# mrluin/TextualDegRemoval

Measured on AMD Instinct MI355X. Metric: train images/sec (512x512, bs=4/GPU), higher is better.
Workload: dtype f32 (3xbf16-split MFMA: 24-bit operand significands on the full fp32 exponent range, fp32 accumulate; unscaled gradients, no loss scale, no step-skip guard; tensors fp32 -- the MASA-encoder ResidualBlock activations / gradients as three bf16 planes whose sum IS the fp32 value, bit for bit)

## Files before the change

include/tdr.h:

```cpp
#ifndef TDR_H
#define TDR_H
#include <stdint.h>
#ifdef __cplusplus
extern "C" {
#endif

#define TDR_ABI_VERSION 112
int tdr_version(void);
const char* tdr_last_error(void);

typedef struct TdrStepGuard {
    float scale, inv_scale, max_scale;
    int good, growth_interval;
    int step, skipped, finite;
    float bc1, bc2_sqrt;
} TdrStepGuard;

typedef struct TdrConvDesc {
    int N, Cin, H, W;
    int Cout, OH, OW;
    int KH, stride, dil, pad;
    const float* in;  int64_t in_ns;
    int gate;
    const float* kscale; int64_t kscale_ns;
// ... 31 lines not shown
    int64_t total;
    int64_t first_block;
} TdrPackJob;
int tdr_pack_job_init(TdrPackJob* job, const float* w, int Cout, int Cin, int KH, int mode, int fmt, void* wp);
int tdr_pack_weights_multi(const TdrPackJob* jobs_dev, int n_jobs, int64_t total_blocks, void* stream);
int tdr_pack_patches(const float* blk, int B, int G, int C, int BH, int BW, int PH, int PW, int pstep, int dil,
                     int off, float* wp, void* stream);

typedef struct TdrConvP16Desc {
    int N, Cin, H, W, Cout;
    const void* in;
    const void* wp; int Mpad; int wp_fmt;
    const float* bias;
    const float* res32;  int64_t res32_ns;
    const void*  res16;
    const float* mask32; int64_t mask32_ns;
    const void*  mask16;
    int relu;
    float* out32; int64_t out32_ns;
    void*  out16;
} TdrConvP16Desc;
int64_t tdr_p16_bytes(int N, int C, int H, int W);
int tdr_p16_from_f32(const float* src, int64_t src_ns, int N, int C, int H, int W, void* dst, void* stream);
int tdr_p16_to_f32(const void* src, int N, int C, int H, int W, float* dst, int64_t dst_ns, void* stream);
int64_t tdr_p16_bytes_fmt(int N, int C, int H, int W, int fmt);
int tdr_p16_from_f32_fmt(const float* src, int64_t src_ns, int N, int C, int H, int W, void* dst, int fmt, void* stream);
int tdr_p16_to_f32_fmt(const void* src, int N, int C, int H, int W, float* dst, int64_t dst_ns, int fmt, void* stream);
int tdr_conv3x3_p16(const TdrConvP16Desc* d, void* stream);
int tdr_conv3x3_p16_force_cfg(int cfg);
typedef struct TdrWgradP16Desc {
    int N, Cin, H, W, Cout;
    const void* in16;
    const void* dout16;
    float* g;
    float* db;
    float* ws; int64_t ws_floats;
    int fmt;
} TdrWgradP16Desc;
int64_t tdr_wgrad3x3_p16_ws_floats(const TdrWgradP16Desc* d);
int tdr_wgrad3x3_p16(const TdrWgradP16Desc* d, void* stream);

typedef struct TdrWgradDesc {
    int N, Cin, H, W, Cout, OH, OW, KH, stride, pad;
    const float* in;   int64_t in_ns;  int gate;
    const float* dout; int64_t dout_ns;
    float* g;
    float* db;
    int per_image;
    float* ws; int64_t ws_floats;
    int math;
} TdrWgradDesc;
int64_t tdr_wgrad_ws_floats(const TdrWgradDesc* d);
int tdr_conv_wgrad(const TdrWgradDesc* d, void* stream);

typedef struct TdrWg1GroupEntry {
    const float* in; const float* dout; float* part; float* dbpart; float* g; float* db;
} TdrWg1GroupEntry;
int tdr_wgrad1x1_group_supported(const TdrWgradDesc* d);
int64_t tdr_wgrad1x1_group_ws_floats(const TdrWgradDesc* d, int nprob);
int tdr_wgrad1x1_group(const TdrWgradDesc* d, int nprob, const void* table, void* stream);

int64_t tdr_wgrad3x3_p16_group_ws_floats(const TdrWgradP16Desc* d, int nprob);
int tdr_wgrad3x3_p16_group_plan(const TdrWgradP16Desc* d, int nprob, int* nsplit, int* units, int* units_per_wg);
int tdr_wgrad3x3_p16_group(const TdrWgradP16Desc* d, int nprob, const void* table, void* stream);

int tdr_layernorm2d_fwd(const float* x, int64_t x_ns, const float* w, const float* b, float eps, int center,
                        int N, int C, int HW, float* y, float* mu, float* rstd, void* stream);
int64_t tdr_ln_ws_floats(int N, int C, int HW);
int tdr_layernorm2d_bwd(const float* go, const float* x, int64_t x_ns, const float* mu, const float* rstd,
                        const float* w, const float* add, int64_t add_ns, int add_C, int center,
                        int N, int C, int HW, float* gx, float* gw, float* gb, float* ws, void* stream);

int64_t tdr_dwsg_ws_floats(int N, int C, int H, int W);
int tdr_dwsg_fwd(const float* t, const float* w, const float* b, int N, int C, int H, int W,
                 float* g, float* pooled, float* ws, void* stream);
int tdr_dwsg_bwd(const float* dg, const float* t, const float* w, const float* b, int N, int C, int H, int W,
                 float* dt, float* dw, float* db, float* ws, void* stream);
int tdr_dwsg_bwd_biased(const float* dg, const float* dg_bias, float dg_bias_mul, const float* t, const float* w, const float* b,
                        int N, int C, int H, int W, float* dt, float* dw, float* db, float* ws, void* stream);
int tdr_dwsg_bwd_parts_supported(int W);
int tdr_dw_param_finish(const float* ws, int N, int C, int H, int W, float* dw , float* db , void* stream);

int tdr_dwgelu_fwd(const float* t, const float* w, const float* b, int N, int C, int H, int W, float* g, void* stream);
int tdr_dwgelu_bwd(const float* dg, const float* t, const float* w, const float* b, int N, int C, int H, int W,
                   float* dt, float* dw, float* db, float* ws, void* stream);
int tdr_dwconv_fwd(const float* t, const float* w, const float* b, int N, int planes, int H, int W, float* out,
                   void* stream);
int tdr_dwconv_bwd(const float* dout, const float* t, const float* w, int N, int planes, int H, int W, float* dt,
                   float* dw, float* db, float* ws, void* stream);
int tdr_dwconv_act_fwd(const float* t, const float* w, const float* b, int N, int planes, int H, int W, int relu, float* out,
                       void* stream);
int tdr_dwconv_act_bwd(const float* dout, const float* act, const float* t, const float* w, int N, int planes, int H, int W,
                       float* dt, float* dw, float* db, float* ws, void* stream);
int tdr_dwpair_fwd(const float* t, const float* w, const float* b, int N, int C, int H, int W, int relu, float* out,
                   int64_t out_ns, void* stream);
int tdr_dwpair_bwd(const float* dout, int64_t dout_ns, const float* act, int64_t act_ns, const float* t, const float* w, int N,
                   int C, int H, int W, float* dt, float* dw, float* db, float* ws, void* stream);
int tdr_dwconv_halves_fwd(const float* t, const float* w, const float* b, int N, int planes, int H, int W, int relu, float* outA,
                          float* outB, int64_t out_ns, void* stream);
int tdr_dwconv_halves_bwd(const float* doutA, const float* doutB, int64_t dout_ns, const float* actA, const float* actB,
                          int64_t act_ns, const float* t, const float* w, int N, int planes, int H, int W, float* dt, float* dw,
                          float* db, float* ws, void* stream);

int tdr_row_sumsq(const float* x, int64_t x_ns, int N, int rows, int HW, float* out, void* stream);
int tdr_mdta_pad(int C);
int tdr_mdta_softmax(const float* G, const float* ss, const float* temp, int N, int C, int heads, float* A, float* AT,
// ... 399 lines not shown
```

textualdegremoval_amd/csrc/tdr_wgrad_1x1.hip:

```cpp
#include "tdr_common.h"
#include "tdr_wgrad_common.h"
#include "../../include/tdr.h"
#include <stdlib.h>

typedef __bf16 g1bf16x8 __attribute__((ext_vector_type(8)));
typedef _Float16 g1f16x8 __attribute__((ext_vector_type(8)));
typedef unsigned g1u32x4 __attribute__((ext_vector_type(4)));

namespace {

enum { G1_BX3 = 0, G1_HX2 = 1 };

constexpr int G1_PX = 32;

template <int SCH>
__device__ __forceinline__ void g1_split8(const f32x4& a, const f32x4& b, g1u32x4 (&p)[SCH == G1_BX3 ? 3 : 2]) {
    if constexpr (SCH == G1_BX3) {
        unsigned h[4], m[4], l[4];
        tdr_split3_bf16<false>(a[0], a[1], h[0], m[0], l[0]);
        tdr_split3_bf16<false>(a[2], a[3], h[1], m[1], l[1]);
        tdr_split3_bf16<false>(b[0], b[1], h[2], m[2], l[2]);
        tdr_split3_bf16<false>(b[2], b[3], h[3], m[3], l[3]);
        p[0] = (g1u32x4){h[0], h[1], h[2], h[3]};
        p[1] = (g1u32x4){m[0], m[1], m[2], m[3]};
// ... 508 lines not shown
    const G1GroupPlan p = g1_group_plan(d, nprob);
    WgArgs a;
    a.in = nullptr; a.in_ns = d->in_ns; a.Cin = d->Cin; a.H = d->H; a.W = d->W;
    a.gate_off = (long)d->Cin * d->H * d->W;
    a.dout = nullptr; a.dout_ns = d->dout_ns; a.Cout = d->Cout; a.OH = d->OH; a.OW = d->OW;
    const G1Tile tl = g1_group_tile(d);
    a.pad = 0; a.tw_log2 = 5; a.tiles_x = tdr_cdiv(d->Cout, 64 * tl.tmw); a.tiles_y = tdr_cdiv(d->Cin, 64 * tl.tnw);
    a.tpi = p.tpi; a.tps = p.tps; a.spi = p.spi;
    a.part = nullptr; a.dbpart = nullptr;
    a.scheme = d->math == 2 ? 1 : 0;
    a.grp_tab = table; a.grp_bpp = p.bpp; a.grp_pairs = nprob * p.bpp;
    hipStream_t st = (hipStream_t)stream;
    const bool g = d->gate != 0;
    int rc;
#define G1_GRP(GATE_, SCH_)                                                                                                       \
    (tl.tmw == 4 ? (tl.tnw == 4 ? launch_grp<GATE_, SCH_, 4, 4>(a, nprob, st) : launch_grp<GATE_, SCH_, 2, 4>(a, nprob, st))      \
                 : (tl.tnw == 2 ? launch_grp<GATE_, SCH_, 2, 2>(a, nprob, st) : launch_grp<GATE_, SCH_, 1, 2>(a, nprob, st)))
    if (a.scheme == 1) rc = g ? G1_GRP(true, G1_HX2) : G1_GRP(false, G1_HX2);
    else rc = g ? G1_GRP(true, G1_BX3) : G1_GRP(false, G1_BX3);
#undef G1_GRP
    if (rc != TDR_OK) return rc;
    const long elems = (long)d->Cout * d->Cin;
    const int nb_main = tdr_cdiv(elems, 256), nb2 = tdr_cdiv(d->Cout, 256);
    hipLaunchKernelGGL(wgrad1x1_grp_reduce_kernel<1>, dim3(nb_main + nb2, nprob), dim3(256), 0, st, static_cast<const TdrWg1GroupEntry*>(table), elems,
                       p.bpp, d->Cout, nb_main);
    TDR_LAUNCH_CHECK("wgrad1x1_grp_reduce_kernel");
    return TDR_OK;
}

namespace {
}

bool tdr_wgrad_1x1_supported(const TdrWgradDesc* d) {
    static const bool off = tdr_tune_env("TDR_WG1") && atoi(tdr_tune_env("TDR_WG1")) == 0;
    if (off || (d->math != 1 && d->math != 2)) return false;
    if (d->KH != 1 || d->stride != 1 || d->pad != 0 || d->H != d->OH || d->W != d->OW) return false;
    const long HW = (long)d->OH * d->OW;
    if (HW % G1_PX != 0 || d->in_ns % 4 != 0 || d->dout_ns % 4 != 0) return false;
    if ((reinterpret_cast<uintptr_t>(d->in) & 15) || (reinterpret_cast<uintptr_t>(d->dout) & 15)) return false;
    return d->Cin >= 64 && d->Cout >= 64;
}

WgPlan tdr_wgrad_1x1_plan(const TdrWgradDesc* d) {
    WgPlan p;
    p.tw_log2 = 5;
    p.cfg = (d->Cout > 64 && d->Cin > 64) ? 0 : 1;
    p.BMc = p.cfg == 0 ? 128 : 64; p.BNc = p.BMc;
    p.WKw = 1;
    const long HW = (long)d->OH * d->OW;
    p.tiles_x = (int)(HW / G1_PX); p.tiles_y = 1;
    p.tpi = p.tiles_x;
    const long out_tiles = (long)tdr_cdiv(d->Cout, p.BMc) * tdr_cdiv(d->Cin, p.BNc);
    static const long want_env = tdr_tune_env("TDR_WG1_WANT") ? atol(tdr_tune_env("TDR_WG1_WANT")) : 0;
    const long want_total = want_env > 0 ? want_env : (d->math == 1 ? 256 : 512);
    long want = want_total / out_tiles;
    if (want < 1) want = 1;
    long spi = (want + d->N - 1) / d->N;
    if (spi > p.tpi / 4) spi = p.tpi / 4;
    if (spi < 1) spi = 1;
    p.tps = tdr_cdiv(p.tpi, spi);
    p.spi = tdr_cdiv(p.tpi, p.tps);
    return p;
}

int tdr_wgrad_1x1_launch(const WgArgs& a, const WgPlan& p, const TdrWgradDesc* d, hipStream_t st) {
    if (p.cfg == 0 && g1_sp() == 1) {
        const bool g = d->gate != 0;
        if (a.scheme == 1) return g ? launch_sp<true, G1_HX2, 2>(a, d->N, st) : launch_sp<false, G1_HX2, 2>(a, d->N, st);
        return g ? launch_sp<true, G1_BX3, 2>(a, d->N, st) : launch_sp<false, G1_BX3, 2>(a, d->N, st);
    }
    if (p.cfg == 0 && g1_sp() == 2) {
        const bool g = d->gate != 0;
        if (a.scheme == 1) return g ? launch_sp<true, G1_HX2, 1>(a, d->N, st) : launch_sp<false, G1_HX2, 1>(a, d->N, st);
        return g ? launch_sp<true, G1_BX3, 1>(a, d->N, st) : launch_sp<false, G1_BX3, 1>(a, d->N, st);
    }
    if (a.scheme == 1) return p.cfg == 0 ? launch_g1_gr<2, 2, G1_HX2>(a, d, st) : launch_g1_gr<1, 1, G1_HX2>(a, d, st);
    return p.cfg == 0 ? launch_g1_gr<2, 2, G1_BX3>(a, d, st) : launch_g1_gr<1, 1, G1_BX3>(a, d, st);
}
```

textualdegremoval_amd/csrc/tdr_wgrad_bx3.hip:

```cpp
#include "tdr_common.h"
#include "tdr_wgrad_common.h"
#include "../../include/tdr.h"

typedef __bf16 bf16x8 __attribute__((ext_vector_type(8)));
typedef _Float16 wf16x8 __attribute__((ext_vector_type(8)));

namespace {

enum { WSCH_BX3 = 0, WSCH_HX2 = 1, WSCH_H1 = 2 };

typedef unsigned u32x4 __attribute__((ext_vector_type(4)));

__device__ __forceinline__ void wsplit3(float x, __bf16& h, __bf16& m, __bf16& l) {
    h = (__bf16)x;
    const float r = x - (float)h;
    m = (__bf16)r;
    l = (__bf16)(r - (float)m);
}

#define WSPLIT_ONE(x, i)                      \
    {                                         \
        __bf16 a0, a1, a2;                    \
        float xp__ = (x);                     \
        asm volatile("" : "+v"(xp__));        \
        wsplit3(xp__, a0, a1, a2);            \
        hv[i] = a0; mv[i] = a1; lv[i] = a2;   \
    }

constexpr int wb_max_nch(int KH, int P) {
    return KH == 3 ? ((P / 32 + 2) * 5 > (P / 8 + 2) * 2 ? ((P / 32 + 2) * 5 > (P / 16 + 2) * 3 ? (P / 32 + 2) * 5 : (P / 16 + 2) * 3)
                                                         : ((P / 8 + 2) * 2 > (P / 16 + 2) * 3 ? (P / 8 + 2) * 2 : (P / 16 + 2) * 3))
                   : P / 8;
}

template <int SCH, bool PIN = true>
__device__ __forceinline__ void split8v(const f32x4& a, const f32x4& b, u32x4& h, u32x4& m, u32x4& l) {
    if constexpr (SCH == WSCH_H1) {
        wf16x8 hv;
#pragma unroll
        for (int i = 0; i < 8; ++i) hv[i] = (_Float16)(i < 4 ? a[i & 3] : b[i & 3]);
        h = __builtin_bit_cast(u32x4, hv);
        m = h;
        l = h;
    } else if constexpr (SCH == WSCH_HX2) {
        unsigned h0, h1, h2, h3, m0, m1, m2, m3;
        tdr_split2_f16<PIN>(a[0], a[1], h0, m0);
        tdr_split2_f16<PIN>(a[2], a[3], h1, m1);
        tdr_split2_f16<PIN>(b[0], b[1], h2, m2);
        tdr_split2_f16<PIN>(b[2], b[3], h3, m3);
        h = (u32x4){h0, h1, h2, h3};
        m = (u32x4){m0, m1, m2, m3};
        l = m;
    } else {
        bf16x8 hv, mv, lv;
        WSPLIT_ONE(a[0], 0) WSPLIT_ONE(a[1], 1) WSPLIT_ONE(a[2], 2) WSPLIT_ONE(a[3], 3)
        WSPLIT_ONE(b[0], 4) WSPLIT_ONE(b[1], 5) WSPLIT_ONE(b[2], 6) WSPLIT_ONE(b[3], 7)
        h = __builtin_bit_cast(u32x4, hv);
        m = __builtin_bit_cast(u32x4, mv);
        l = __builtin_bit_cast(u32x4, lv);
    }
}

template <int KH, int P, int WMw, int WNw, int WKw, int TMW, int TNW, bool GATE, bool PRE, bool DMA, int CL, int SCH>
__global__ __launch_bounds__(256, 2) void wgrad_bx3_kernel(WgArgs a) {
    constexpr int NS = SCH == WSCH_BX3 ? 3 : (SCH == WSCH_HX2 ? 2 : 1);
    constexpr int NP = SCH == WSCH_BX3 ? 6 : (SCH == WSCH_HX2 ? 3 : 1);
    static_assert(!DMA || (KH == 3 && !PRE && !GATE), "DMA staging: 3x3 only");
    static_assert(WMw * WNw * WKw == 4, "4 waves");
    static_assert(KH == 1 || (TMW == 1 && TNW == 1), "3x3: one 32x32 tile pair (9 accumulators) per wave");
    constexpr int TAPS = KH * KH;
    constexpr int BMc = 32 * TMW * WMw, BNc = 32 * TNW * WNw;
    constexpr int HALO = KH == 3 ? 1 : 0;
    constexpr int DCH = P / 8;
    constexpr int NITD = (BMc * DCH + 255) / 256;
    constexpr int NITI = (BNc * (((P >> CL) + (KH == 3 ? 2 : 0)) * ((KH == 3 ? (1 << CL) + 8 : (1 << CL)) >> 3)) + 255) / 256;
    constexpr int KSTEPS = P / 16;
    constexpr int KPW = KSTEPS / WKw;
    static_assert(KPW >= 1, "tile too small for the K split");
    constexpr int DPITCH = P + 8;

    extern __shared__ __attribute__((aligned(16))) unsigned char smem_raw[];
    const int tid = threadIdx.x, lane = tid & 63, wave = __builtin_amdgcn_readfirstlane(tid >> 6);
    const int wk = wave % WKw, wn = (wave / WKw) % WNw, wm = wave / (WKw * WNw);
    const int j = lane & 31, kg = lane >> 5;
    constexpr int cl = CL, C = 1 << cl, R = P >> cl;
    static_assert(R >= 1, "tile narrower than its width");
    constexpr int CP = KH == 3 ? C + 8 : C;
    constexpr int LR = R + 2 * HALO;
    constexpr int NCH = (LR * CP) >> 3;
    constexpr int IPITCH = (NCH | 1) << 3;
    __bf16* s_d = reinterpret_cast<__bf16*>(smem_raw);
    __bf16* s_i = s_d + NS * BMc * DPITCH;
    float* raw_d = reinterpret_cast<float*>(s_i + NS * BNc * IPITCH);
    float* raw_i = raw_d + BMc * P;

    const int split = blockIdx.x;
    const int n = split / a.spi;
    const int t_begin = (split % a.spi) * a.tps;
    const int t_end = min(t_begin + a.tps, a.tpi);
    const int co0 = blockIdx.y * BMc, ci0 = blockIdx.z * BNc;
    const long HWin = (long)a.H * a.W, HWo = (long)a.OH * a.OW;
    const float* in_n = a.in + (long)n * a.in_ns;
    const float* do_n = a.dout + (long)n * a.dout_ns;

    float dsum[NITD];
#pragma unroll
    for (int i = 0; i < NITD; ++i) dsum[i] = 0.f;

    const f32x4 z4 = {0.f, 0.f, 0.f, 0.f};
    auto tile_origin = [&](int t, int& oy0, int& ox0, int& ty) {
        int tx;
        if (KH == 3) { tx = t / a.tiles_y; ty = t - tx * a.tiles_y; }
        else { ty = t / a.tiles_x; tx = t - ty * a.tiles_x; }
        oy0 = ty * R;
        ox0 = tx * C;
    };
    auto d_load = [&](int t, int it, f32x4& v0, f32x4& v1, int& ldsoff, bool& live, bool from_raw = false) {
        int oy0, ox0, ty;
        tile_origin(t, oy0, ox0, ty);
        const int id = tid + 256 * it;
        live = (BMc * DCH % 256 == 0) || id < BMc * DCH;
        const int idc = min(id, BMc * DCH - 1);
        const int col = idc / DCH, ch = idc - col * DCH;
        const int row = (ch * 8) >> cl, xo = (ch * 8) & (C - 1);
        const int oy = oy0 + row, ox = ox0 + xo;
        const int co = min(co0 + col, a.Cout - 1);
        const bool rok = oy < a.OH && co0 + col < a.Cout;
        const float* src = do_n + (long)co * HWo + (long)min(oy, a.OH - 1) * a.OW;
        const bool ok0 = rok && ox < a.OW, ok1 = rok && ox + 4 < a.OW;
        if (DMA && from_raw) {
            v0 = *reinterpret_cast<const f32x4*>(raw_d + idc * 8);
            v1 = *reinterpret_cast<const f32x4*>(raw_d + idc * 8 + 4);
        } else {
            v0 = *reinterpret_cast<const f32x4*>(src + (ok0 ? ox : 0));
            v1 = *reinterpret_cast<const f32x4*>(src + (ok1 ? ox + 4 : 0));
        }
        ldsoff = (col * DPITCH + ch * 8) | (ok0 ? 1 << 30 : 0) | (ok1 ? (int)0x80000000u : 0);
    };
    auto d_store = [&](int it, const f32x4& r0, const f32x4& r1, int ldsoff_, bool live) {
        if (!live) return;
        const f32x4 v0 = (ldsoff_ >> 30) & 1 ? r0 : z4, v1 = ((unsigned)ldsoff_ >> 31) ? r1 : z4;
        const int ldsoff = ldsoff_ & 0x3fffffff;
        dsum[it] += ((v0[0] + v0[1]) + (v0[2] + v0[3])) + ((v1[0] + v1[1]) + (v1[2] + v1[3]));
        u32x4 h, m, l;
        split8v<SCH, false>(v0, v1, h, m, l);
        u32x4* dst = reinterpret_cast<u32x4*>(s_d + ldsoff);
        dst[0] = h;
        if constexpr (NS >= 2) dst[(BMc * DPITCH) >> 3] = m;
        if constexpr (NS == 3) dst[(2 * BMc * DPITCH) >> 3] = l;
    };
    auto i_load = [&](int t, int it, f32x4& v0, f32x4& v1, f32x4& g0, f32x4& g1, int& ldsoff, bool& live, bool from_raw = false) {
        int oy0, ox0, ty;
        tile_origin(t, oy0, ox0, ty);
        const int lr0 = (KH == 3 && t != t_begin && ty != 0) ? 2 : 0;
        constexpr int CPR = CP >> 3;
        const int nchr = (LR - lr0) * CPR;
        const int id = tid + 256 * it;
        live = id < BNc * nchr;
        const int idc = min(id, BNc * nchr - 1);
        const int cil = idc / nchr, rem = idc - cil * nchr;
        const int lrow = lr0 + rem / CPR, c0 = (rem % CPR) * 8;
        const int slot = KH == 3 ? (oy0 + lrow) % LR : lrow;
        const int gy = oy0 - a.pad + lrow;
        const int gx0 = KH == 3 ? ox0 + c0 - 4 : ox0 + c0;
        const int ci = min(ci0 + cil, a.Cin - 1);
        const bool rok = gy >= 0 && gy < a.H && ci0 + cil < a.Cin;
        const float* src = in_n + (long)ci * HWin + (long)min(max(gy, 0), a.H - 1) * a.W;
        const bool ok0 = rok && gx0 >= 0 && gx0 < a.W, ok1 = rok && gx0 + 4 >= 0 && gx0 + 4 < a.W;
        const int o0 = ok0 ? gx0 : 0, o1 = ok1 ? gx0 + 4 : 0;
        if (DMA && from_raw) {
            v0 = *reinterpret_cast<const f32x4*>(raw_i + idc * 8);
            v1 = *reinterpret_cast<const f32x4*>(raw_i + idc * 8 + 4);
        } else {
            v0 = *reinterpret_cast<const f32x4*>(src + o0);
            v1 = *reinterpret_cast<const f32x4*>(src + o1);
        }
        if (GATE) {
            g0 = *reinterpret_cast<const f32x4*>(src + o0 + a.gate_off);
            g1 = *reinterpret_cast<const f32x4*>(src + o1 + a.gate_off);
        }
        ldsoff = (cil * IPITCH + slot * CP + c0) | (ok0 ? 1 << 30 : 0) | (ok1 ? (int)0x80000000u : 0);
    };
    auto i_store = [&](const f32x4& r0, const f32x4& r1, const f32x4& g0, const f32x4& g1, int ldsoff_, bool live) {
        if (!live) return;
        const f32x4 v0 = (ldsoff_ >> 30) & 1 ? (GATE ? r0 * g0 : r0) : z4, v1 = ((unsigned)ldsoff_ >> 31) ? (GATE ? r1 * g1 : r1) : z4;
        const int ldsoff = ldsoff_ & 0x3fffffff;
        u32x4 h, m, l;
        split8v<SCH, GATE>(v0, v1, h, m, l);
        u32x4* dst = reinterpret_cast<u32x4*>(s_i + ldsoff);
        dst[0] = h;
        if constexpr (NS >= 2) dst[(BNc * IPITCH) >> 3] = m;
        if constexpr (NS == 3) dst[(2 * BNc * IPITCH) >> 3] = l;
    };
    f32x4 pd0[PRE ? NITD : 1], pd1[PRE ? NITD : 1], pi0[PRE ? NITI : 1], pi1[PRE ? NITI : 1];
    f32x4 pg0[PRE && GATE ? NITI : 1], pg1[PRE && GATE ? NITI : 1];
    int pdo[PRE ? NITD : 1], pio[PRE ? NITI : 1];
    bool pdl[PRE ? NITD : 1], pil[PRE ? NITI : 1];
    auto prefetch = [&](int t) {
        if constexpr (PRE) {
#pragma unroll
            for (int it = 0; it < NITD; ++it) d_load(t, it, pd0[it], pd1[it], pdo[it], pdl[it]);
#pragma unroll
            for (int it = 0; it < NITI; ++it) i_load(t, it, pi0[it], pi1[it], pg0[GATE ? it : 0], pg1[GATE ? it : 0], pio[it], pil[it]);
        }
    };
    auto commit = [&]() {
        if constexpr (PRE) {
#pragma unroll
            for (int it = 0; it < NITD; ++it) d_store(it, pd0[it], pd1[it], pdo[it], pdl[it]);
#pragma unroll
            for (int it = 0; it < NITI; ++it) i_store(pi0[it], pi1[it], pg0[GATE ? it : 0], pg1[GATE ? it : 0], pio[it], pil[it]);
        }
    };
    auto stage_sync = [&](int t, bool from_raw = false) {
#pragma unroll
        for (int it = 0; it < NITD; ++it) {
            f32x4 v0, v1; int o; bool live;
            d_load(t, it, v0, v1, o, live, from_raw);
            d_store(it, v0, v1, o, live);
        }
#pragma unroll
        for (int it = 0; it < NITI; ++it) {
            f32x4 v0, v1, g0 = z4, g1 = z4; int o; bool live;
            i_load(t, it, v0, v1, g0, g1, o, live, from_raw);
            i_store(v0, v1, g0, g1, o, live);
        }
    };
    auto steady = [&](int t) {
        int oy0, ox0, ty;
        tile_origin(t, oy0, ox0, ty);
        return KH == 3 && t != t_begin && ty != 0;
    };
    auto dma_issue = [&](int t) {
        if constexpr (DMA) {
            int oy0, ox0, ty;
            tile_origin(t, oy0, ox0, ty);
            constexpr int DP = BMc * P / 4;
#pragma unroll
            for (int k = 0; k < (DP + 255) / 256; ++k) {
                const int id = tid + 256 * k;
                if (DP % 256 == 0 || id < DP) {
                    const int col = id / (P / 4), c4 = id - col * (P / 4);
                    const int row = (c4 * 4) >> cl, xo = (c4 * 4) & (C - 1);
                    const int oy = min(oy0 + row, a.OH - 1), ox = ox0 + xo;
                    const float* g = do_n + (long)min(co0 + col, a.Cout - 1) * HWo + (long)oy * a.OW + (ox < a.OW ? ox : 0);
                    float* l = raw_d + __builtin_amdgcn_readfirstlane((wave * 64 + 256 * k) * 4);
                    __builtin_amdgcn_global_load_lds((__attribute__((address_space(1))) const void*)g,
                                                     (__attribute__((address_space(3))) void*)l, 16, 0, 0);
                }
            }
            constexpr int CPQ = CP >> 2, per_c = R * CPQ, IP = BNc * per_c;
            for (int k = 0; k * 256 < IP; ++k) {
                const int id = tid + 256 * k;
                if (id < IP) {
                    const int cil = id / per_c, rem = id - cil * per_c;
                    const int lrow = 2 + rem / CPQ, q = rem % CPQ;
                    const int gy = min(max(oy0 - a.pad + lrow, 0), a.H - 1), gx = ox0 - 4 + 4 * q;
                    const float* g = in_n + (long)min(ci0 + cil, a.Cin - 1) * HWin + (long)gy * a.W + ((gx >= 0 && gx < a.W) ? gx : 0);
                    float* l = raw_i + __builtin_amdgcn_readfirstlane((wave * 64 + 256 * k) * 4);
                    __builtin_amdgcn_global_load_lds((__attribute__((address_space(1))) const void*)g,
                                                     (__attribute__((address_space(3))) void*)l, 16, 0, 0);
                }
            }
        }
    };

    f32x16 acc[TMW][TNW][TAPS];
#pragma unroll
    for (int x = 0; x < TMW; ++x)
#pragma unroll
        for (int y = 0; y < TNW; ++y)
#pragma unroll
            for (int t = 0; t < TAPS; ++t)
#pragma unroll
                for (int r = 0; r < 16; ++r) acc[x][y][t][r] = 0.f;
// ... 83 lines not shown
            a.dbpart[(long)split * a.Cout + co0 + tid] = s;
        }
    }
    if constexpr (WKw > 1) {
        float* red = reinterpret_cast<float*>(smem_raw) + (wave / WKw) * (TMW * TNW * TAPS * 16 * 64);
#pragma unroll
        for (int w = 1; w < WKw; ++w) {
            __syncthreads();
            if (wk == w) {
#pragma unroll
                for (int x = 0; x < TMW; ++x)
#pragma unroll
                    for (int y = 0; y < TNW; ++y)
#pragma unroll
                        for (int t = 0; t < TAPS; ++t)
#pragma unroll
                            for (int r = 0; r < 16; ++r) red[(((x * TNW + y) * TAPS + t) * 16 + r) * 64 + lane] = acc[x][y][t][r];
            }
            __syncthreads();
            if (wk == 0) {
#pragma unroll
                for (int x = 0; x < TMW; ++x)
#pragma unroll
                    for (int y = 0; y < TNW; ++y)
#pragma unroll
                        for (int t = 0; t < TAPS; ++t)
#pragma unroll
                            for (int r = 0; r < 16; ++r) acc[x][y][t][r] += red[(((x * TNW + y) * TAPS + t) * 16 + r) * 64 + lane];
            }
        }
        if (wk != 0) return;
    }
    float* part = a.part + (long)split * a.Cout * a.Cin * TAPS;
#pragma unroll
    for (int x = 0; x < TMW; ++x)
#pragma unroll
        for (int y = 0; y < TNW; ++y) {
            const int ci = ci0 + (wn * TNW + y) * 32 + j;
            if (ci >= a.Cin) continue;
#pragma unroll
            for (int r = 0; r < 16; ++r) {
                const int co = co0 + (wm * TMW + x) * 32 + (r & 3) + 8 * (r >> 2) + 4 * kg;
                if (co >= a.Cout) continue;
#pragma unroll
                for (int tap = 0; tap < TAPS; ++tap) part[((long)co * a.Cin + ci) * TAPS + tap] = acc[x][y][tap][r];
            }
        }
}

template <int KH, int P, int WMw, int WNw, int WKw, int TMW, int TNW, bool GATE, bool PRE, bool DMA, int CL, int SCH>
int launch_wgb_cl_s(const WgArgs& a, const WgPlan& p, int N, hipStream_t st) {
    constexpr int NS = SCH == WSCH_BX3 ? 3 : (SCH == WSCH_HX2 ? 2 : 1);
    constexpr int BMc = 32 * TMW * WMw, BNc = 32 * TNW * WNw;
    constexpr int C = 1 << CL, R = P / C;
    constexpr int CP = KH == 3 ? C + 8 : C, LR = KH == 3 ? R + 2 : R;
    constexpr int ipitch = (((LR * CP) >> 3) | 1) << 3;
    size_t lds = (size_t)(NS * BMc * (P + 8) + NS * BNc * ipitch) * 2 + (DMA ? (size_t)(BMc * P + BNc * R * CP) * 4 : 0);
    const size_t red = (size_t)(WKw > 1 ? (4 / WKw) * TMW * TNW * KH * KH * 16 * 64 : BMc * (P / 8)) * 4;
    if (lds < red) lds = red;
    dim3 grid(N * p.spi, tdr_cdiv(a.Cout, BMc), tdr_cdiv(a.Cin, BNc));
    auto kern = wgrad_bx3_kernel<KH, P, WMw, WNw, WKw, TMW, TNW, GATE, PRE, DMA, CL, SCH>;
    static bool attr_set = false;
    if (!attr_set) {
        (void)hipFuncSetAttribute(reinterpret_cast<const void*>(kern), hipFuncAttributeMaxDynamicSharedMemorySize, 160 * 1024);
        attr_set = true;
    }
    hipLaunchKernelGGL(kern, grid, dim3(256), lds, st, a);
    TDR_LAUNCH_CHECK("wgrad_bx3_kernel");
    return TDR_OK;
}

template <int KH, int P, int WMw, int WNw, int WKw, int TMW, int TNW, bool GATE, bool PRE, bool DMA, int CL>
int launch_wgb_cl(const WgArgs& a, const WgPlan& p, int N, hipStream_t st) {
    if (a.scheme == WSCH_HX2) return launch_wgb_cl_s<KH, P, WMw, WNw, WKw, TMW, TNW, GATE, PRE, DMA, CL, WSCH_HX2>(a, p, N, st);
    if (a.scheme == WSCH_H1) return launch_wgb_cl_s<KH, P, WMw, WNw, WKw, TMW, TNW, GATE, PRE, DMA, CL, WSCH_H1>(a, p, N, st);
    return launch_wgb_cl_s<KH, P, WMw, WNw, WKw, TMW, TNW, GATE, PRE, DMA, CL, WSCH_BX3>(a, p, N, st);
}

template <int KH, int P, int WMw, int WNw, int WKw, int TMW, int TNW, bool GATE, bool PRE, bool DMA = false>
int launch_wgb(const WgArgs& a, const WgPlan& p, int N, hipStream_t st) {
    if (a.tw_log2 == 5) return launch_wgb_cl<KH, P, WMw, WNw, WKw, TMW, TNW, GATE, PRE, DMA, 5>(a, p, N, st);
    if (a.tw_log2 == 4) return launch_wgb_cl<KH, P, WMw, WNw, WKw, TMW, TNW, GATE, PRE, DMA, 4>(a, p, N, st);
    return launch_wgb_cl<KH, P, WMw, WNw, WKw, TMW, TNW, GATE, PRE, DMA, 3>(a, p, N, st);
}

}

bool tdr_wgrad_bx3_supported(const TdrWgradDesc* d) {
    if (d->stride != 1 || d->OW < 8 || d->W % 4 != 0 || d->OW % 4 != 0) return false;
    if (d->in_ns % 4 != 0 || d->dout_ns % 4 != 0) return false;
    if (d->KH == 1) return d->pad == 0;
    return d->KH == 3 && d->pad == 1 && !d->gate;
}

WgPlan tdr_wgrad_bx3_plan(const TdrWgradDesc* d) {
    WgPlan p;
    p.tw_log2 = d->OW >= 24 ? 5 : (d->OW >= 12 ? 4 : 3);
    if (d->KH == 1) {
        static const int force1 = tdr_tune_env("TDR_WGB_CFG1X1") ? atoi(tdr_tune_env("TDR_WGB_CFG1X1")) : -1;
        if (force1 >= 0 && d->Cout >= 64 && d->Cin >= 64) p.cfg = force1;
        else if (d->Cout > 64 && d->Cin > 64) p.cfg = 0;
        else if (d->Cin <= 32 && d->Cout <= 32) p.cfg = 2;
        else if (d->Cin <= 32) p.cfg = 5;
        else p.cfg = 1;
    } else {
        p.cfg = (d->Cin <= 32 && d->Cout <= 32) ? 4 : 3;
    }
    static const int bm[6] = {128, 64, 32, 64, 32, 64}, bn[6] = {128, 64, 32, 64, 32, 32};
    static const int pp[6] = {32, 64, 128, 32, 128, 64};
    p.BMc = bm[p.cfg]; p.BNc = bn[p.cfg];
    p.WKw = 1;
    const int P = pp[p.cfg];
    const int C = 1 << p.tw_log2, R = P / C;
    p.tiles_x = tdr_cdiv(d->OW, C);
    p.tiles_y = tdr_cdiv(d->OH, R);
    p.tpi = p.tiles_x * p.tiles_y;
    const long out_tiles = (long)tdr_cdiv(d->Cout, p.BMc) * tdr_cdiv(d->Cin, p.BNc);
    static const long want_env = tdr_tune_env("TDR_WG_WANT") ? atol(tdr_tune_env("TDR_WG_WANT")) : 0;
    const long want_total = want_env > 0 ? want_env : (d->math == 1 ? 256 : 512);
    long want = want_total / out_tiles;
    if (want < 1) want = 1;
    long spi = (want + d->N - 1) / d->N;
    if (spi > p.tpi / 4) spi = p.tpi / 4;
    if (spi < 1) spi = 1;
    p.tps = tdr_cdiv(p.tpi, spi);
    p.spi = tdr_cdiv(p.tpi, p.tps);
    return p;
}

int tdr_wgrad_bx3_launch(const WgArgs& a, const WgPlan& p, const TdrWgradDesc* d, hipStream_t st) {
    const bool g = d->gate != 0;
    switch (p.cfg) {
        case 0: return g ? launch_wgb<1, 32, 2, 2, 1, 2, 2, true, true>(a, p, d->N, st) : launch_wgb<1, 32, 2, 2, 1, 2, 2, false, true>(a, p, d->N, st);
        case 1: return g ? launch_wgb<1, 64, 2, 2, 1, 1, 1, true, true>(a, p, d->N, st) : launch_wgb<1, 64, 2, 2, 1, 1, 1, false, true>(a, p, d->N, st);
        case 2: return g ? launch_wgb<1, 128, 1, 1, 4, 1, 1, true, true>(a, p, d->N, st) : launch_wgb<1, 128, 1, 1, 4, 1, 1, false, true>(a, p, d->N, st);
        case 3: return launch_wgb<3, 32, 2, 2, 1, 1, 1, false, false, true>(a, p, d->N, st);
        case 4: return launch_wgb<3, 128, 1, 1, 4, 1, 1, false, false>(a, p, d->N, st);
        default: return g ? launch_wgb<1, 64, 2, 1, 2, 1, 1, true, true>(a, p, d->N, st) : launch_wgb<1, 64, 2, 1, 2, 1, 1, false, true>(a, p, d->N, st);
    }
}
```

textualdegremoval_amd/csrc/tdr_wgrad_common.h:

```cpp
#pragma once
#include "tdr_common.h"

struct TdrWgradDesc;

struct WgArgs {
    const float* in; long in_ns; int Cin, H, W; long gate_off;
    const float* dout; long dout_ns; int Cout, OH, OW;
    int pad, tw_log2, tiles_x, tiles_y, tpi , tps , spi ;
    float* part;
    float* dbpart;
    int scheme;
    const void* grp_tab;
    int grp_bpp;
    int grp_pairs;
};

struct WgPlan { int tw_log2, tiles_x, tiles_y, tpi, tps, spi, cfg, WKw, BMc, BNc; };

bool tdr_wgrad_bx3_supported(const TdrWgradDesc* d);
WgPlan tdr_wgrad_bx3_plan(const TdrWgradDesc* d);
int tdr_wgrad_bx3_launch(const WgArgs& a, const WgPlan& p, const TdrWgradDesc* d, hipStream_t st);

bool tdr_wgrad_s2_supported(const TdrWgradDesc* d);
WgPlan tdr_wgrad_s2_plan(const TdrWgradDesc* d);
int tdr_wgrad_s2_launch(const WgArgs& a, const WgPlan& p, const TdrWgradDesc* d, hipStream_t st);

bool tdr_wgrad_1x1_supported(const TdrWgradDesc* d);
WgPlan tdr_wgrad_1x1_plan(const TdrWgradDesc* d);
int tdr_wgrad_1x1_launch(const WgArgs& a, const WgPlan& p, const TdrWgradDesc* d, hipStream_t st);
```

textualdegremoval_amd/csrc/tdr_wgrad_mfma.hip:

```cpp
#include <stdio.h>
#include <stdlib.h>
#include "tdr_common.h"
#include "tdr_wgrad_common.h"
#include "../../include/tdr.h"

namespace {

constexpr int wg_plane(int TW, int KH, int S) { return (((64 / TW) - 1) * S + KH) * ((TW - 1) * S + KH); }
constexpr int wg_cmax(int a, int b) { return a > b ? a : b; }
constexpr int wg_max_plane(int KH, int S) {
    return wg_cmax(wg_plane(8, KH, S), wg_cmax(wg_plane(16, KH, S), wg_plane(32, KH, S)));
}

template <int KH, int S, int WMw, int WNw, int WKw, int TMW, int TNW, bool GATE>
__global__ __launch_bounds__(256) void wgrad_mfma_kernel(WgArgs a) {
    static_assert(WMw * WNw * WKw == 4, "4 waves");
    constexpr int TAPS = KH * KH;
    constexpr int BMc = 32 * TMW * WMw, BNc = 32 * TNW * WNw;
    constexpr int MAXPIT = (wg_max_plane(KH, S) + 63) / 64;
    constexpr int DPT = BMc / 4;
    constexpr int IPT = BNc / 4;
    constexpr int KPW = 32 / WKw;

    extern __shared__ __attribute__((aligned(16))) float smem[];
// ... 184 lines not shown
    if (d->math >= 1 && tdr_wgrad_bx3_supported(d)) return tdr_wgrad_bx3_plan(d);
    if (tdr_wgrad_s2_supported(d)) return tdr_wgrad_s2_plan(d);
    WgPlan p;
    p.tw_log2 = d->OW >= 24 ? 5 : (d->OW >= 12 ? 4 : 3);
    const int TW = 1 << p.tw_log2, TH = 64 >> p.tw_log2;
    p.tiles_x = tdr_cdiv(d->OW, TW);
    p.tiles_y = tdr_cdiv(d->OH, TH);
    p.tpi = p.tiles_x * p.tiles_y;
    if (d->KH == 1) {
        if (d->Cout >= 128 && d->Cin >= 128) p.cfg = 0;
        else if (d->Cin <= 32) p.cfg = d->Cout <= 32 ? 3 : 1;
        else p.cfg = 2;
    } else if (d->KH == 3 && d->stride == 1) {
        p.cfg = (d->Cin <= 32 && d->Cout <= 32) ? 3 : 2;
    } else {
        p.cfg = 2;
    }
    static const int bm[4] = {128, 64, 64, 32}, bn[4] = {128, 32, 64, 32}, wk[4] = {1, 4, 1, 4};
    p.BMc = bm[p.cfg]; p.BNc = bn[p.cfg]; p.WKw = wk[p.cfg];
    const long out_tiles = (long)tdr_cdiv(d->Cout, p.BMc) * tdr_cdiv(d->Cin, p.BNc);
    long want = (p.WKw > 1 ? 256 : 512) / out_tiles;
    if (want < 1) want = 1;
    long spi = (want + d->N - 1) / d->N;
    if (spi > p.tpi / 4) spi = p.tpi / 4;
    if (spi < 1) spi = 1;
    p.tps = tdr_cdiv(p.tpi, spi);
    p.spi = tdr_cdiv(p.tpi, p.tps);
    return p;
}

template <int KH, int S, int WMw, int WNw, int WKw, int TMW, int TNW, bool GATE>
int launch_wg(const WgArgs& a, const WgPlan& p, int N, hipStream_t st) {
    constexpr int BMc = 32 * TMW * WMw, BNc = 32 * TNW * WNw;
    const int TW = 1 << a.tw_log2;
    const int LH = ((64 >> a.tw_log2) - 1) * S + KH, LW = (TW - 1) * S + KH;
    const size_t lds = (size_t)(BMc * 65 + BNc * ((LH * LW) | 1)) * sizeof(float);
    dim3 grid(N * p.spi, tdr_cdiv(a.Cout, BMc), tdr_cdiv(a.Cin, BNc));
    auto kern = wgrad_mfma_kernel<KH, S, WMw, WNw, WKw, TMW, TNW, GATE>;
    static bool attr_set = false;
    if (!attr_set) {
        (void)hipFuncSetAttribute(reinterpret_cast<const void*>(kern), hipFuncAttributeMaxDynamicSharedMemorySize, 160 * 1024);
        attr_set = true;
    }
    hipLaunchKernelGGL(kern, grid, dim3(256), lds, st, a);
    TDR_LAUNCH_CHECK("wgrad_mfma_kernel");
    return TDR_OK;
}

}

extern "C" int64_t tdr_wgrad_ws_floats(const TdrWgradDesc* d) {
    const WgPlan p = make_plan(d);
    return (int64_t)d->N * p.spi * p.WKw * d->Cout * d->Cin * d->KH * d->KH + (int64_t)d->N * p.spi * d->Cout;
}

extern "C" int tdr_conv_wgrad(const TdrWgradDesc* d, void* stream) {
    TDR_REQUIRE(d && d->in && d->dout && d->g && d->ws, "tdr_conv_wgrad: null pointer");
    const WgPlan p = make_plan(d);
    const int64_t need = tdr_wgrad_ws_floats(d);
    TDR_REQUIRE(d->ws_floats >= need, "tdr_conv_wgrad: workspace too small (%lld < %lld)", (long long)d->ws_floats,
                (long long)need);
    WgArgs a;
    a.in = d->in; a.in_ns = d->in_ns; a.Cin = d->Cin; a.H = d->H; a.W = d->W;
    a.gate_off = (long)d->Cin * d->H * d->W;
    a.dout = d->dout; a.dout_ns = d->dout_ns; a.Cout = d->Cout; a.OH = d->OH; a.OW = d->OW;
    a.grp_tab = nullptr; a.grp_bpp = 0; a.grp_pairs = 0;
    a.pad = d->pad; a.tw_log2 = p.tw_log2; a.tiles_x = p.tiles_x; a.tiles_y = p.tiles_y; a.tpi = p.tpi; a.tps = p.tps; a.spi = p.spi;
    const bool direct = !d->db && (d->per_image ? p.spi : d->N * p.spi) * p.WKw == 1;
    a.part = direct ? d->g : d->ws;
    a.dbpart = d->db ? d->ws + (int64_t)d->N * p.spi * p.WKw * d->Cout * d->Cin * d->KH * d->KH : nullptr;
    hipStream_t st = (hipStream_t)stream;
    const bool g = d->gate != 0;
    int rc = TDR_ERR_UNSUPPORTED;
    const int key = d->KH * 10 + d->stride;
    a.scheme = d->math == 3 ? 2 : (d->math == 2 ? 1 : 0);
    static const bool dbg = tdr_tune_env("TDR_WG_DEBUG") != nullptr;
    if (dbg && !(d->math >= 1 && tdr_wgrad_bx3_supported(d)) && !tdr_wgrad_s2_supported(d))
        fprintf(stderr, "[tdr] exact wgrad: math %d N %d %d->%d @%dx%d k%d s%d pad %d gate %d per_image %d in_ns %ld dout_ns %ld\n", d->math,
                d->N, d->Cin, d->Cout, d->H, d->W, d->KH, d->stride, d->pad, d->gate, d->per_image, (long)d->in_ns, (long)d->dout_ns);
    if (tdr_wgrad_1x1_supported(d)) {
        rc = tdr_wgrad_1x1_launch(a, p, d, st);
    } else if (d->math >= 1 && tdr_wgrad_bx3_supported(d)) {
        rc = tdr_wgrad_bx3_launch(a, p, d, st);
    } else if (tdr_wgrad_s2_supported(d)) {
        rc = tdr_wgrad_s2_launch(a, p, d, st);
    } else if (key == 11) {
        switch (p.cfg) {
            case 0: rc = g ? launch_wg<1, 1, 2, 2, 1, 2, 2, true>(a, p, d->N, st) : launch_wg<1, 1, 2, 2, 1, 2, 2, false>(a, p, d->N, st); break;
            case 1: rc = g ? launch_wg<1, 1, 1, 1, 4, 2, 1, true>(a, p, d->N, st) : launch_wg<1, 1, 1, 1, 4, 2, 1, false>(a, p, d->N, st); break;
            case 2: rc = g ? launch_wg<1, 1, 2, 2, 1, 1, 1, true>(a, p, d->N, st) : launch_wg<1, 1, 2, 2, 1, 1, 1, false>(a, p, d->N, st); break;
            default: rc = g ? launch_wg<1, 1, 1, 1, 4, 1, 1, true>(a, p, d->N, st) : launch_wg<1, 1, 1, 1, 4, 1, 1, false>(a, p, d->N, st); break;
        }
    } else if (key == 31 && !g) {
        rc = p.cfg == 3 ? launch_wg<3, 1, 1, 1, 4, 1, 1, false>(a, p, d->N, st) : launch_wg<3, 1, 2, 2, 1, 1, 1, false>(a, p, d->N, st);
    } else if (key == 32 && !g) {
        rc = launch_wg<3, 2, 2, 2, 1, 1, 1, false>(a, p, d->N, st);
    } else if (key == 22 && !g) {
        rc = launch_wg<2, 2, 2, 2, 1, 1, 1, false>(a, p, d->N, st);
    } else {
        tdr_set_error("tdr_conv_wgrad: unsupported (KH=%d stride=%d gate=%d)", d->KH, d->stride, d->gate);
        return TDR_ERR_UNSUPPORTED;
    }
    if (rc != TDR_OK || direct) return rc;
    const long elems = (long)d->Cout * d->Cin * d->KH * d->KH;
    const int groups = d->per_image ? d->N : 1;
    const int per_group = (d->per_image ? p.spi : d->N * p.spi) * p.WKw;
// ... 17 lines not shown
```

Baseline: 60.96.

## Size narrow-channel wgrad grids to CU residency and trim padded channel tiles

For narrow weight-gradient problems (at most 64 channels, few output tiles), the split-K planner now sets the total workgroup count from an estimate of how many blocks fit per CU, based on LDS footprint and register limits capped by an env knob. Previously it used a fixed target of 256 or 512. In the 3x3 bx3 kernel, partially filled channel tiles (e.g. 3 input channels) now zero the LDS planes once and skip loads and stores for dead channels. The goal is fewer wasted loads for tiny channel counts and a full wave of resident blocks, in exchange for more partial-sum reduction and hardcoded CU and LDS constants. A plan-query API and a probe script are also added.

New measurement: 61.37, median of 6. No clear change (+0.7%).

```diff
diff --git a/include/tdr.h b/include/tdr.h
--- a/include/tdr.h
+++ b/include/tdr.h
@@ -107,6 +107,7 @@
 } TdrWgradDesc;
 int64_t tdr_wgrad_ws_floats(const TdrWgradDesc* d);
 int tdr_conv_wgrad(const TdrWgradDesc* d, void* stream);
+int tdr_wgrad_plan(const TdrWgradDesc* d, int* family, int* cfg, int* spi, int* tps, int* resident);
 
 typedef struct TdrWg1GroupEntry {
     const float* in; const float* dout; float* part; float* dbpart; float* g; float* db;
diff --git a/profiles/wgrad_narrow/probe_wgrad_narrow.py b/profiles/wgrad_narrow/probe_wgrad_narrow.py
--- /dev/null
+++ b/profiles/wgrad_narrow/probe_wgrad_narrow.py
@@ -0,0 +1,54 @@
+import ctypes as C
+import os
+import sys
+
+import torch
+
+sys.path.insert(0, os.path.dirname(os.path.dirname(os.path.dirname(os.path.abspath(__file__)))))
+from textualdegremoval_amd import _lib, kernels as K
+
+SHAPES = [(4, 3, 32, 512, 512, 3, False), (8, 3, 32, 512, 512, 3, False), (4, 32, 3, 512, 512, 3, False),
+          (4, 32, 32, 512, 512, 1, False), (4, 32, 32, 512, 512, 1, True), (4, 32, 64, 512, 512, 1, False),
+          (4, 32, 64, 512, 512, 1, True), (4, 64, 64, 256, 256, 1, False), (4, 64, 64, 256, 256, 1, True)]
+
+
+def plan(lib, N, Cin, Cout, H, W, KH, gate):
+    if not hasattr(lib, 'tdr_wgrad_plan'):
+        return None
+    d = _lib.TdrWgradDesc()
+    d.N, d.Cin, d.H, d.W, d.Cout, d.OH, d.OW = N, Cin, H, W, Cout, H, W
+    d.KH, d.stride, d.pad = KH, 1, KH // 2
+    d.in_ns, d.dout_ns, d.gate, d.math = Cin * (2 if gate else 1) * H * W, Cout * H * W, 1 if gate else 0, 1
+    out = [C.c_int() for _ in range(5)]
+    lib.tdr_wgrad_plan(C.byref(d), *[C.byref(o) for o in out])
+    return tuple(o.value for o in out)
+
+
+def main():
+    reps = int(sys.argv[1]) if len(sys.argv) > 1 else 20
+    K.set_math('bx3')
+    lib = _lib.load()
+    total = 0.0
+    for N, Cin, Cout, H, W, KH, gate in SHAPES:
+        x = torch.randn(N, Cin * (2 if gate else 1), H, W, device='cuda')
+        d = torch.randn(N, Cout, H, W, device='cuda')
+        for _ in range(3):
+            K.conv_wgrad(x, d, Cout, Cin, KH, pad=KH // 2, gate=gate, want_db=True)
+        t0, t1 = torch.cuda.Event(enable_timing=True), torch.cuda.Event(enable_timing=True)
+        torch.cuda.synchronize()
+        t0.record()
+        for _ in range(reps):
+            K.conv_wgrad(x, d, Cout, Cin, KH, pad=KH // 2, gate=gate, want_db=True)
+        t1.record()
+        torch.cuda.synchronize()
+        us = t0.elapsed_time(t1) * 1e3 / reps
+        total += us
+        gb = (x.numel() + d.numel()) * 4 / 1e9
+        p = plan(lib, N, Cin, Cout, H, W, KH, gate)
+        wgs = f'{N * p[2]:5d} workgroups (family {p[0]} cfg {p[1]}, {p[4]} per CU)' if p else ''
+        print(f'{Cin:3d}->{Cout:3d} k{KH} N{N} {H}x{W}{" gate" if gate else "     "}: {us:8.1f} us  {gb / us * 1e6:7.0f} GB/s  {wgs}')
+    print(f'sum {total:8.1f} us')
+
+
+if __name__ == '__main__':
+    main()
diff --git a/textualdegremoval_amd/csrc/tdr_wgrad_1x1.hip b/textualdegremoval_amd/csrc/tdr_wgrad_1x1.hip
--- a/textualdegremoval_amd/csrc/tdr_wgrad_1x1.hip
+++ b/textualdegremoval_amd/csrc/tdr_wgrad_1x1.hip
@@ -584,7 +584,17 @@
     p.tpi = p.tiles_x;
     const long out_tiles = (long)tdr_cdiv(d->Cout, p.BMc) * tdr_cdiv(d->Cin, p.BNc);
     static const long want_env = tdr_tune_env("TDR_WG1_WANT") ? atol(tdr_tune_env("TDR_WG1_WANT")) : 0;
-    const long want_total = want_env > 0 ? want_env : (d->math == 1 ? 256 : 512);
+    long want_total = want_env > 0 ? want_env : (d->math == 1 ? 256 : 512);
+    p.resident = 0;
+    const int cap = tdr_wg_narrow_cap();
+    if (want_env <= 0 && cap > 0 && d->math == 1 && !d->per_image && p.cfg == 1 && d->Cout == 64 && d->Cin == 64) {
+        const int ring_lds = g1_ring() * (64 + (d->gate ? 2 : 1) * 64) * 128;
+        int res = TDR_WG_LDS_PER_CU / ring_lds;
+        if (res > 5) res = 5;
+        if (res > cap) res = cap;
+        p.resident = res;
+        want_total = (long)TDR_WG_CUS * res;
+    }
     long want = want_total / out_tiles;
     if (want < 1) want = 1;
     long spi = (want + d->N - 1) / d->N;
diff --git a/textualdegremoval_amd/csrc/tdr_wgrad_bx3.hip b/textualdegremoval_amd/csrc/tdr_wgrad_bx3.hip
--- a/textualdegremoval_amd/csrc/tdr_wgrad_bx3.hip
+++ b/textualdegremoval_amd/csrc/tdr_wgrad_bx3.hip
@@ -31,6 +31,15 @@
     return KH == 3 ? ((P / 32 + 2) * 5 > (P / 8 + 2) * 2 ? ((P / 32 + 2) * 5 > (P / 16 + 2) * 3 ? (P / 32 + 2) * 5 : (P / 16 + 2) * 3)
                                                          : ((P / 8 + 2) * 2 > (P / 16 + 2) * 3 ? (P / 8 + 2) * 2 : (P / 16 + 2) * 3))
                    : P / 8;
+}
+
+constexpr size_t wgb_lds_bytes(int KH, int P, int BMc, int BNc, int WKw, int TT, int NS, int CL, bool DMA) {
+    const int C = 1 << CL, R = P / C;
+    const int CP = KH == 3 ? C + 8 : C, LR = KH == 3 ? R + 2 : R;
+    const int ipitch = (((LR * CP) >> 3) | 1) << 3;
+    const size_t lds = (size_t)(NS * BMc * (P + 8) + NS * BNc * ipitch) * 2 + (DMA ? (size_t)(BMc * P + BNc * R * CP) * 4 : 0);
+    const size_t red = (size_t)(WKw > 1 ? (4 / WKw) * TT * KH * KH * 16 * 64 : BMc * (P / 8)) * 4;
+    return lds < red ? red : lds;
 }
 
 template <int SCH, bool PIN = true>
@@ -106,6 +115,13 @@
     float dsum[NITD];
 #pragma unroll
     for (int i = 0; i < NITD; ++i) dsum[i] = 0.f;
+    constexpr bool TRIM = KH == 3 && !PRE && !DMA;
+    const int nco = TRIM ? min(BMc, a.Cout - co0) : BMc, nci = TRIM ? min(BNc, a.Cin - ci0) : BNc;
+    if (TRIM && (nco < BMc || nci < BNc)) {
+        constexpr int Z16 = (NS * BMc * DPITCH + NS * BNc * IPITCH) / 8;
+        static_assert((NS * BMc * DPITCH + NS * BNc * IPITCH) % 8 == 0, "plane tiles are whole 16-byte pieces");
+        for (int i = tid; i < Z16; i += 256) reinterpret_cast<u32x4*>(smem_raw)[i] = (u32x4){0u, 0u, 0u, 0u};
+    }
 
     const f32x4 z4 = {0.f, 0.f, 0.f, 0.f};
     auto tile_origin = [&](int t, int& oy0, int& ox0, int& ty) {
@@ -119,7 +135,7 @@
         int oy0, ox0, ty;
         tile_origin(t, oy0, ox0, ty);
         const int id = tid + 256 * it;
-        live = (BMc * DCH % 256 == 0) || id < BMc * DCH;
+        live = TRIM ? id < nco * DCH : ((BMc * DCH % 256 == 0) || id < BMc * DCH);
         const int idc = min(id, BMc * DCH - 1);
         const int col = idc / DCH, ch = idc - col * DCH;
         const int row = (ch * 8) >> cl, xo = (ch * 8) & (C - 1);
@@ -156,7 +172,7 @@
         constexpr int CPR = CP >> 3;
         const int nchr = (LR - lr0) * CPR;
         const int id = tid + 256 * it;
-        live = id < BNc * nchr;
+        live = id < (TRIM ? nci : BNc) * nchr;
         const int idc = min(id, BNc * nchr - 1);
         const int cil = idc / nchr, rem = idc - cil * nchr;
         const int lrow = lr0 + rem / CPR, c0 = (rem % CPR) * 8;
@@ -213,14 +229,19 @@
         }
     };
     auto stage_sync = [&](int t, bool from_raw = false) {
+        int oy0_, ox0_, ty_;
+        tile_origin(t, oy0_, ox0_, ty_);
+        const int ilim = TRIM ? nci * ((LR - ((t != t_begin && ty_ != 0) ? 2 : 0)) * (CP >> 3)) : 0;
 #pragma unroll
         for (int it = 0; it < NITD; ++it) {
+            if (TRIM && 256 * it >= nco * DCH) break;
             f32x4 v0, v1; int o; bool live;
             d_load(t, it, v0, v1, o, live, from_raw);
             d_store(it, v0, v1, o, live);
         }
 #pragma unroll
         for (int it = 0; it < NITI; ++it) {
+            if (TRIM && 256 * it >= ilim) break;
             f32x4 v0, v1, g0 = z4, g1 = z4; int o; bool live;
             i_load(t, it, v0, v1, g0, g1, o, live, from_raw);
             i_store(v0, v1, g0, g1, o, live);
@@ -410,12 +431,7 @@
 int launch_wgb_cl_s(const WgArgs& a, const WgPlan& p, int N, hipStream_t st) {
     constexpr int NS = SCH == WSCH_BX3 ? 3 : (SCH == WSCH_HX2 ? 2 : 1);
     constexpr int BMc = 32 * TMW * WMw, BNc = 32 * TNW * WNw;
-    constexpr int C = 1 << CL, R = P / C;
-    constexpr int CP = KH == 3 ? C + 8 : C, LR = KH == 3 ? R + 2 : R;
-    constexpr int ipitch = (((LR * CP) >> 3) | 1) << 3;
-    size_t lds = (size_t)(NS * BMc * (P + 8) + NS * BNc * ipitch) * 2 + (DMA ? (size_t)(BMc * P + BNc * R * CP) * 4 : 0);
-    const size_t red = (size_t)(WKw > 1 ? (4 / WKw) * TMW * TNW * KH * KH * 16 * 64 : BMc * (P / 8)) * 4;
-    if (lds < red) lds = red;
+    constexpr size_t lds = wgb_lds_bytes(KH, P, BMc, BNc, WKw, TMW * TNW, NS, CL, DMA);
     dim3 grid(N * p.spi, tdr_cdiv(a.Cout, BMc), tdr_cdiv(a.Cin, BNc));
     auto kern = wgrad_bx3_kernel<KH, P, WMw, WNw, WKw, TMW, TNW, GATE, PRE, DMA, CL, SCH>;
     static bool attr_set = false;
@@ -475,7 +491,19 @@
     p.tpi = p.tiles_x * p.tiles_y;
     const long out_tiles = (long)tdr_cdiv(d->Cout, p.BMc) * tdr_cdiv(d->Cin, p.BNc);
     static const long want_env = tdr_tune_env("TDR_WG_WANT") ? atol(tdr_tune_env("TDR_WG_WANT")) : 0;
-    const long want_total = want_env > 0 ? want_env : (d->math == 1 ? 256 : 512);
+    long want_total = want_env > 0 ? want_env : (d->math == 1 ? 256 : 512);
+    p.resident = 0;
+    const int cap = tdr_wg_narrow_cap();
+    if (want_env <= 0 && cap > 0 && d->math == 1 && !d->per_image && out_tiles <= 4 && d->Cout <= 64 && d->Cin <= 64 && p.cfg != 0 && p.cfg != 3) {
+        static const int wkw[6] = {1, 1, 4, 1, 4, 2}, by_regs[6][2] = {{2, 2}, {4, 3}, {4, 3}, {2, 2}, {2, 2}, {4, 4}};
+        const size_t lds = wgb_lds_bytes(d->KH, P, p.BMc, p.BNc, wkw[p.cfg], 1, 3, p.tw_log2, false);
+        int res = (int)(TDR_WG_LDS_PER_CU / lds);
+        if (res > by_regs[p.cfg][d->gate ? 1 : 0]) res = by_regs[p.cfg][d->gate ? 1 : 0];
+        if (res > cap) res = cap;
+        if (res < 1) res = 1;
+        p.resident = res;
+        want_total = (long)TDR_WG_CUS * res;
+    }
     long want = want_total / out_tiles;
     if (want < 1) want = 1;
     long spi = (want + d->N - 1) / d->N;
diff --git a/textualdegremoval_amd/csrc/tdr_wgrad_common.h b/textualdegremoval_amd/csrc/tdr_wgrad_common.h
--- a/textualdegremoval_amd/csrc/tdr_wgrad_common.h
+++ b/textualdegremoval_amd/csrc/tdr_wgrad_common.h
@@ -15,7 +15,17 @@
     int grp_pairs;
 };
 
-struct WgPlan { int tw_log2, tiles_x, tiles_y, tpi, tps, spi, cfg, WKw, BMc, BNc; };
+struct WgPlan {
+    int tw_log2, tiles_x, tiles_y, tpi, tps, spi, cfg, WKw, BMc, BNc;
+    int resident = 0;
+};
+
+constexpr int TDR_WG_CUS = 256;
+constexpr int TDR_WG_LDS_PER_CU = 160 * 1024;
+inline int tdr_wg_narrow_cap() {
+    static const int cap = tdr_tune_env("TDR_WG_NARROW") ? atoi(tdr_tune_env("TDR_WG_NARROW")) : 4;
+    return cap;
+}
 
 bool tdr_wgrad_bx3_supported(const TdrWgradDesc* d);
 WgPlan tdr_wgrad_bx3_plan(const TdrWgradDesc* d);
diff --git a/textualdegremoval_amd/csrc/tdr_wgrad_mfma.hip b/textualdegremoval_amd/csrc/tdr_wgrad_mfma.hip
--- a/textualdegremoval_amd/csrc/tdr_wgrad_mfma.hip
+++ b/textualdegremoval_amd/csrc/tdr_wgrad_mfma.hip
@@ -260,6 +260,14 @@
 extern "C" int64_t tdr_wgrad_ws_floats(const TdrWgradDesc* d) {
     const WgPlan p = make_plan(d);
     return (int64_t)d->N * p.spi * p.WKw * d->Cout * d->Cin * d->KH * d->KH + (int64_t)d->N * p.spi * d->Cout;
+}
+
+extern "C" int tdr_wgrad_plan(const TdrWgradDesc* d, int* family, int* cfg, int* spi, int* tps, int* resident) {
+    TDR_REQUIRE(d && family && cfg && spi && tps && resident, "tdr_wgrad_plan: null pointer");
+    const WgPlan p = make_plan(d);
+    *family = tdr_wgrad_1x1_supported(d) ? 2 : ((d->math >= 1 && tdr_wgrad_bx3_supported(d)) ? 1 : (tdr_wgrad_s2_supported(d) ? 3 : 0));
+    *cfg = p.cfg; *spi = p.spi; *tps = p.tps; *resident = p.resident;
+    return TDR_OK;
 }
 
 extern "C" int tdr_conv_wgrad(const TdrWgradDesc* d, void* stream) {
```
